# wdas03/lipreading-video-generation

Measured on AMD Instinct MI355X. Metric: train-step frames/sec + DDIM steps/sec, 128x128x16 UNet3D at 1/2/4/8 GPUs, higher is better.
Workload: dtype bf16

## Files before the change

### include/vdiff.h

```cpp
#ifndef VDIFF_H
#define VDIFF_H

#include <stdint.h>
#include <stddef.h>

#ifdef __cplusplus
extern "C" {
#endif

#define VDIFF_ABI_VERSION 1

enum vd_status { VD_OK = 0, VD_EINVAL = 1, VD_EUNSUPPORTED = 2, VD_ELAUNCH = 3 };
enum vd_dtype { VD_F32 = 0, VD_BF16 = 1 };

int vd_version(void);
const char* vd_last_error(void);
int vd_device_info(char* buf, int buflen);

int vd_timestep_embedding(const int64_t* t, int B, int dim, float max_period,
                          float* out, void* stream);
int vd_timestep_embedding_tab(const int64_t* t, int B, int dim, const float* freqs,
                              float* out, void* stream);

int vd_q_sample(const void* x0, const void* eps, void* xt, const int64_t* t,
                const float* sqrt_acp, const float* sqrt_1m_acp,
                int64_t B, int64_t per_sample, int dtype, void* stream);

// ... 16 lines not shown
                   int64_t B, int64_t per_sample, int dtype, void* stream);

int vd_p_sample_cosine(const void* xt, const void* eps, const void* z,
                       void* x_prev, void* mean_out, const int64_t* t,
                       const float* acp, const float* sqrt_acp,
                       const float* sqrt_1m_acp, int64_t B, int64_t per_sample,
                       int dtype, void* stream);

int vd_ddim_step(const void* xt, const void* eps, const void* z, void* x_prev,
                 void* x0, const int64_t* t, const int64_t* t_prev,
                 const float* acp, float eta, int clip, int64_t B,
                 int64_t per_sample, int dtype, void* stream);

void vd_set_dropout_counter(const uint64_t* counter);
int vd_groupnorm_set_unroll(int u);
size_t vd_groupnorm_workspace_size(int B, int64_t S, int C, int G);
int vd_groupnorm_silu_fwd(const void* x, const float* gamma, const float* beta,
                          void* y, float* mean, float* rstd, int B, int64_t S,
                          int C, int G, float eps, int silu, float drop_p,
                          uint64_t seed, int dtype, void* workspace,
                          void* stream);
int vd_groupnorm_silu_bwd(const void* x, const void* dy, const float* gamma,
                          const float* beta, const float* mean,
                          const float* rstd, void* dx, float* dgamma,
                          float* dbeta, int B, int64_t S, int C, int G,
                          int silu, float drop_p, uint64_t seed, int dtype,
                          void* workspace, void* stream);
int vd_groupnorm_silu_bwd_add(const void* x, const void* dy, const void* dadd,
                              const float* gamma, const float* beta, const float* mean,
                              const float* rstd, void* dx, float* dgamma, float* dbeta,
// ... 30 lines not shown
  int dtype;
} vd_conv_desc;

int vd_conv3d_fwd(const vd_conv_desc* d, const void* x, const void* w_fwd,
                  const float* bias, const float* chan_add,
                  const void* residual, void* y, void* stream);
int vd_conv3d_bwd_data(const vd_conv_desc* d, const void* dy,
                       const void* w_bwd, void* dx, void* stream);
int vd_conv3d_bwd_weight(const vd_conv_desc* d, const void* x, const void* dy,
                         float* dw, void* stream);
size_t vd_conv3d_bwd_weight_workspace_size(const vd_conv_desc* d);
int vd_conv3d_bwd_weight_det(const vd_conv_desc* d, const void* x, const void* dy, float* dw,
                             int Co_out, int Ci_out, void* workspace, size_t workspace_bytes,
                             void* stream);

int vd_conv_set_wgrad(int mode);
int vd_conv_set_halo(int mode);

size_t vd_channel_sums_workspace_size(int B, int C);
int vd_channel_sums(const void* x, int B, int64_t S, int C, int cstride, int dtype,
                    float* out, void* workspace, void* stream);
int vd_conv_pack_weight(const float* w, int Co, int Ci, int taps, int Cip, int Cop,
                        int transpose, int dtype, void* out, void* stream);
typedef struct {
  const float* w;
  void* out;
  int Co, Ci, taps, Cip, Cop, transpose;
  int64_t start;
} vd_pack_desc;
int vd_conv_pack_weights(const vd_pack_desc* descs, int n, int64_t total, int dtype,
                         void* stream);

// ... 76 lines not shown
```

### lipreading-video-generation_amd/csrc/conv.hip

```cpp
#include "vd_common.h"
#include <stdio.h>
#include <stdlib.h>

#include <atomic>

namespace {

constexpr int kThreads = 256;
constexpr int kBK = 32;

template <typename T> struct Cfg;
template <> struct Cfg<bf16_t> {
  static constexpr int EPC = 8;
  static constexpr int CPR = kBK / EPC;
  static constexpr int LDK = kBK;
};
template <> struct Cfg<float> {
  static constexpr int EPC = 4;
  static constexpr int CPR = kBK / EPC;
  static constexpr int LDK = kBK + 4;
};

__device__ __forceinline__ int swz(int r, int kc) {
  const int t = (r >> 2) & 3;
// ... 1700 lines not shown
int halo_ks(const GemmGeom& g, bool ) {
  if (conv_halo_mode() == 0 || !halo_ok(g)) return 0;
  static const int force = [] {
    const char* e = getenv("VDIFF_CONV_HALO_KS");
    return e ? atoi(e) : 0;
  }();
  if (force == 32 || force == 64) return force;
  return (g.dW <= 32 || g.sC >= 128) ? 64 : 32;
}
template <bool TR, int KS, int NW, bool EA = true, bool EH = false>
void launch_halo_tile(const GemmGeom& g, const void* src, const void* wt, void* dst,
                  const float* bias, const float* ca, const void* res, hipStream_t st) {
  const size_t lds_c = (size_t)kHoT * NW * kHoW * (64 + 4) * 4;
  const size_t lds = halo_lds<3, KS, NW>() > lds_c ? halo_lds<3, KS, NW>() : lds_c;
  auto kern = halo_conv_kernel<TR, KS, NW, EA, EH>;
  (void)hipFuncSetAttribute((const void*)kern, hipFuncAttributeMaxDynamicSharedMemorySize,
                            (int)lds);
  const int64_t tiles = (int64_t)g.B * vd_cdiv(g.dT, kHoT) * vd_cdiv(g.dH, NW) * (g.dW / kHoW);
  dim3 grid((unsigned)tiles, (unsigned)vd_cdiv(g.N, 64));
  kern<<<grid, 64 * NW, lds, st>>>(g, (const bf16_t*)src, (const bf16_t*)wt, (bf16_t*)dst, bias,
                                   ca, (const bf16_t*)res);
}
template <bool TR>
void launch_halo(const GemmGeom& g, int ks, const void* src, const void* wt, void* dst,
                 const float* bias, const float* ca, const void* res, hipStream_t st) {
  if (conv_halo_mode() == 3) {
    if (ks == 32) launch_halo_tile<TR, 32, 8>(g, src, wt, dst, bias, ca, res, st);
    else launch_halo_tile<TR, 64, 8>(g, src, wt, dst, bias, ca, res, st);
    return;
  }
  if (conv_halo_mode() == 4) {
    if (ks == 32) launch_halo_tile<TR, 32, 4, false>(g, src, wt, dst, bias, ca, res, st);
// ... 1 lines not shown
    return;
  }
  if constexpr (!TR) {
    if (conv_halo_mode() != 5) {
      if (ks == 32) launch_halo_tile<TR, 32, 4, true, true>(g, src, wt, dst, bias, ca, res, st);
      else launch_halo_tile<TR, 64, 4, true, true>(g, src, wt, dst, bias, ca, res, st);
      return;
    }
  }
  if (ks == 32) launch_halo_tile<TR, 32, 4>(g, src, wt, dst, bias, ca, res, st);
  else launch_halo_tile<TR, 64, 4>(g, src, wt, dst, bias, ca, res, st);
}

constexpr int kPwMaxLds = 40 * 1024;

template <int KS>
__global__ __launch_bounds__(256) void pw_gemm_kernel(
    const bf16_t* __restrict__ src, int sCs, const bf16_t* __restrict__ wt, int N, int NS,
    bf16_t* __restrict__ dst, int dNs, const float* __restrict__ bias,
    const float* __restrict__ chan_add, int64_t ppb, const bf16_t* __restrict__ residual,
    int64_t M) {
  constexpr int K = 32 * KS, RS = K + 8;
  extern __shared__ __attribute__((aligned(16))) char smem[];
  bf16_t* wl = reinterpret_cast<bf16_t*>(smem);
  const int tid = threadIdx.x, lane = tid & 63;
  const int wave = __builtin_amdgcn_readfirstlane(tid >> 6);
  const int nbase = blockIdx.y * NS;
  const int nsl = N - nbase < NS ? N - nbase : NS;
  const int nrow = (nsl + 63) / 64 * 64;
  for (int c = tid; c < nrow * (K / 8); c += 256) {
    const int r = c / (K / 8), k8 = c % (K / 8);
    *reinterpret_cast<uint4*>(wl + r * RS + k8 * 8) =
        r < nsl ? *reinterpret_cast<const uint4*>(wt + (int64_t)(nbase + r) * K + k8 * 8)
                : make_uint4(0, 0, 0, 0);
  }
  __syncthreads();

  const int fr = lane & 15, fq = lane >> 4;
  const int64_t ntiles = (M + 15) / 16;
  const int64_t stride = (int64_t)gridDim.x * 4;
  auto load = [&](bf16x8 (&x)[KS], int64_t tile) __attribute__((always_inline)) {
    const int64_t p = tile * 16 + fr;
    const bool ok = tile < ntiles && p < M;
    const bf16_t* row = src + (ok ? p : 0) * (int64_t)sCs + 8 * fq;
#pragma unroll
    for (int kk = 0; kk < KS; ++kk) {
      const uint4 v = ok ? *reinterpret_cast<const uint4*>(row + 32 * kk) : make_uint4(0, 0, 0, 0);
      x[kk] = __builtin_bit_cast(bf16x8, v);
    }
  };
  bf16x8 xc[KS], xn[KS];
  int64_t tile = (int64_t)blockIdx.x * 4 + wave;
  load(xc, tile);
  for (; tile < ntiles; tile += stride) {
    load(xn, tile + stride);
    const int64_t p = tile * 16 + fr;
    const bool pok = p < M;
    const int b = chan_add ? (int)((pok ? p : 0) / ppb) : 0;
    bf16_t* out = dst + (pok ? p : 0) * (int64_t)dNs + nbase;
    const bf16_t* res = residual ? residual + (pok ? p : 0) * (int64_t)dNs + nbase : nullptr;
    for (int n0 = 0; n0 < nsl; n0 += 64) {
      f32x4 acc[4];
#pragma unroll
      for (int j = 0; j < 4; ++j) acc[j] = f32x4{0.f, 0.f, 0.f, 0.f};
#pragma unroll
      for (int j = 0; j < 4; ++j) {
        const bf16_t* wr = wl + (n0 + 16 * (fr >> 2) + 4 * j + (fr & 3)) * RS + 8 * fq;
#pragma unroll
// ... 32 lines not shown
#pragma unroll
            for (int e = 0; e < 8; ++e) o[8 * h + e] += rv[e];
          }
        }
#pragma unroll
        for (int h = 0; h < 2; ++h) {
          float v8[8];
#pragma unroll
          for (int e = 0; e < 8; ++e) v8[e] = o[8 * h + e];
          store8(out + nl + 8 * h, v8);
        }
      }
    }
#pragma unroll
    for (int kk = 0; kk < KS; ++kk) xc[kk] = xn[kk];
  }
}

int pw_gemm_launch(const GemmGeom& g, const void* src, const void* wt, void* dst,
                   const float* bias, const float* ca, const void* res, hipStream_t st) {
  const int K = g.sC;
  if (g.kt * g.kh * g.kw != 1 || g.st != 1 || g.sh != 1 || g.sw != 1 || g.pt || g.ph || g.pw)
    return -1;
  if (K % 32 || K > 256 || g.N % 16 || g.sCs % 8 || g.dNs % 8 || g.K != K) return -1;
  if ((reinterpret_cast<uintptr_t>(src) & 15) || (reinterpret_cast<uintptr_t>(wt) & 15) ||
      (reinterpret_cast<uintptr_t>(dst) & 15) || (reinterpret_cast<uintptr_t>(res) & 15))
    return -1;
  if (bias && (reinterpret_cast<uintptr_t>(bias) & 15)) return -1;
  if (ca && ((reinterpret_cast<uintptr_t>(ca) & 15) || g.N % 4)) return -1;
  const int row_bytes = (K + 8) * 2;
  int NS = (kPwMaxLds / row_bytes) / 64 * 64;
  if (NS < 64) return -1;
  int slices = (int)vd_cdiv(g.N, NS);
  NS = (int)vd_cdiv(vd_cdiv(g.N, slices), 64) * 64;
  slices = (int)vd_cdiv(g.N, NS);
  const size_t lds = (size_t)NS * row_bytes;
  const int64_t tiles = vd_cdiv(g.M, 16);
  int64_t wgs = vd_cdiv(tiles, 4);
  const int64_t cap = (int64_t)256 * 4 / slices;
  if (wgs > cap) wgs = cap < 256 ? 256 : cap;
  const int64_t ppb = (int64_t)g.dT * g.dH * g.dW;
  dim3 grid((unsigned)wgs, (unsigned)slices);
#define VD_PW_CASE(KS_)                                                                          \
  case KS_: {                                                                                    \
    auto kern = pw_gemm_kernel<KS_>;                                                             \
    (void)hipFuncSetAttribute((const void*)kern, hipFuncAttributeMaxDynamicSharedMemorySize,     \
                              (int)lds);                                                         \
    kern<<<grid, 256, lds, st>>>((const bf16_t*)src, g.sCs, (const bf16_t*)wt, g.N, NS,          \
                                 (bf16_t*)dst, g.dNs, bias, ca, ppb, (const bf16_t*)res, g.M);   \
    return VD_OK;                                                                                \
  }
  switch (K / 32) {
    VD_PW_CASE(1) VD_PW_CASE(2) VD_PW_CASE(3) VD_PW_CASE(4)
    VD_PW_CASE(5) VD_PW_CASE(6) VD_PW_CASE(7) VD_PW_CASE(8)
  }
#undef VD_PW_CASE
  return -1;
}

#ifndef VD_PW_DEFAULT
#define VD_PW_DEFAULT 1
#endif
const bool g_conv_pw = [] {
  const char* e = getenv("VDIFF_CONV_PW");
  return e ? atoi(e) != 0 : VD_PW_DEFAULT != 0;
}();

int conv_1x1_variant() {
  static const int v = [] {
    const char* e = getenv("VDIFF_CONV_1X1");
    return e ? atoi(e) : 3;
// ... 103 lines not shown
  VD_REQUIRE(x && w_fwd && y, "null tensor");
  GemmGeom g;
  g.B = d->B;
  g.sT = d->Ti; g.sH = d->Hi; g.sW = d->Wi; g.sC = d->Ci;
  g.sCs = d->x_cstride ? d->x_cstride : d->Ci;
  g.dT = d->To; g.dH = d->Ho; g.dW = d->Wo; g.N = d->Co;
  g.dNs = d->y_cstride ? d->y_cstride : d->Co;
  g.kt = d->kt; g.kh = d->kh; g.kw = d->kw;
  g.st = d->st; g.sh = d->sh; g.sw = d->sw;
  g.pt = d->pt; g.ph = d->ph; g.pw = d->pw;
  g.M = (int64_t)d->B * d->To * d->Ho * d->Wo;
  g.K = d->kt * d->kh * d->kw * d->Ci;
  return VD_DISPATCH_DTYPE(d->dtype, T, {
    launch_gemm<T, false>(g, x, w_fwd, y, bias, chan_add, residual, VD_STREAM(stream));
  });
}

int vd_conv_set_wgrad(int mode) {
  if (mode < 0 || mode > 2) {
    (void)vd::fail(VD_EINVAL, "conv wgrad mode %d (0, 1, 2)", mode);
    return -2;
  }
  return g_wgrad_mode.exchange(mode);
}

int vd_conv_set_halo(int mode) {
  if (mode < 0 || mode > 5) {
    (void)vd::fail(VD_EINVAL, "conv halo mode %d (0 - 5)", mode);
    return -2;
  }
// ... 345 lines not shown
```

### lipreading-video-generation_amd/csrc/groupnorm.hip

```cpp
#include <atomic>

#include "vd_common.h"

namespace {

constexpr int kThreads = 256;
constexpr int kVec = 8;
static int env_int(const char* name, int dflt) {
  const char* e = getenv(name);
  const int v = e ? atoi(e) : 0;
  return v > 0 ? v : dflt;
}
const int kTargetChunks = env_int("VDIFF_GN_CHUNKS", 1024);
const int kSumPer = env_int("VDIFF_GN_SUMPER", 64);
std::atomic<int> g_gn_unroll{env_int("VDIFF_GN_UNROLL", 2)};

struct GNPlan {
  int rows_per_iter;
  int64_t chunk_px;
  int nchunk;
};

inline GNPlan gn_plan(int B, int64_t S, int C) {
  GNPlan p;
  const int nvec = C / kVec;
  p.rows_per_iter = kThreads / nvec;
  if (p.rows_per_iter < 1) p.rows_per_iter = 1;
  int64_t want = vd_cdiv(S * B, kTargetChunks);
  if (want < p.rows_per_iter) want = p.rows_per_iter;
  want = vd_cdiv(want, p.rows_per_iter) * p.rows_per_iter;
  p.chunk_px = want;
  p.nchunk = (int)vd_cdiv(S, want);
  return p;
}

struct Stat {
  float n, m, q;
};
__device__ __forceinline__ Stat chan(Stat a, Stat b) {
  const float n = a.n + b.n;
  if (n == 0.f) return a;
  const float d = b.m - a.m;
  const float fb = b.n / n;
  Stat r;
  r.n = n;
  r.m = a.m + d * fb;
  r.q = a.q + b.q + d * d * a.n * fb;
  return r;
}

struct Drop {
  float p, inv_keep;
  uint64_t seed;
  const uint64_t* ctr;
  __device__ __forceinline__ Drop resolved() const {
    Drop d = *this;
    if (p > 0.f && ctr) d.seed = seed ^ ((*ctr + 1) * 0x9E3779B97F4A7C15ull);
    d.ctr = nullptr;
    return d;
  }
  __device__ __forceinline__ float mul(int64_t idx) const {
    return p > 0.f ? dropout_mul(seed, idx, p, inv_keep) : 1.f;
  }
};
// ... 126 lines not shown
                                                            const float* __restrict__ beta,
                                                            const float* __restrict__ mean,
                                                            const float* __restrict__ rstd,
                                                            T* __restrict__ y, int64_t S, int C,
                                                            int G, int64_t chunk_px,
                                                            int rows_per_iter, Drop drop_in) {
  const Drop drop = drop_in.resolved();
  const int nvec = C / kVec, cpg = C / G;
  const int b = blockIdx.y, tid = threadIdx.x;
  const int r = tid / nvec, cv = tid % nvec;
  if (r >= rows_per_iter) return;
  float sc[kVec], sh[kVec];
#pragma unroll
  for (int j = 0; j < kVec; ++j) {
    const int c = cv * kVec + j, g = b * G + c / cpg;
    sc[j] = gamma[c] * rstd[g];
    sh[j] = beta[c] - mean[g] * sc[j];
  }
  const int64_t p0 = (int64_t)blockIdx.x * chunk_px;
  int64_t p1 = p0 + chunk_px;
  if (p1 > S) p1 = S;
  int64_t p = p0 + r;
  if constexpr (U > 1) {
    for (; p + (U - 1) * rows_per_iter < p1; p += U * rows_per_iter) {
      float v[U][kVec];
#pragma unroll
      for (int u = 0; u < U; ++u)
        load8(x + ((int64_t)b * S + p + u * rows_per_iter) * C + cv * kVec, v[u]);
#pragma unroll
      for (int u = 0; u < U; ++u) {
        const int64_t e0 = ((int64_t)b * S + p + u * rows_per_iter) * C + cv * kVec;
#pragma unroll
        for (int j = 0; j < kVec; ++j) {
          const float z = v[u][j] * sc[j] + sh[j];
          v[u][j] = (SILU ? silu_f(z) : z) * drop.mul(e0 + j);
        }
        store8(y + e0, v[u]);
      }
    }
  }
  for (; p < p1; p += rows_per_iter) {
    const int64_t e0 = ((int64_t)b * S + p) * C + cv * kVec;
    float v[kVec];
    load8(x + e0, v);
#pragma unroll
    for (int j = 0; j < kVec; ++j) {
      const float z = v[j] * sc[j] + sh[j];
      v[j] = (SILU ? silu_f(z) : z) * drop.mul(e0 + j);
    }
    store8(y + e0, v);
  }
}

template <typename T, bool SILU, int U>
__global__ __launch_bounds__(kThreads) void gn_bwd_reduce_kernel(
    const T* __restrict__ x, const T* __restrict__ dy, const float* __restrict__ gamma,
    const float* __restrict__ beta, const float* __restrict__ mean, const float* __restrict__ rstd,
    int64_t S, int C, int G, int64_t chunk_px, int rows_per_iter, float* __restrict__ part,
    Drop drop_in) {
  const Drop drop = drop_in.resolved();
  extern __shared__ __attribute__((aligned(16))) char smem[];
  float2* sh = reinterpret_cast<float2*>(smem);
// ... 220 lines not shown
}


int gn_check(const void* x, int B, int64_t S, int C, int G) {
  VD_REQUIRE(x, "null tensor");
  VD_REQUIRE(B > 0 && S > 0 && C > 0 && G > 0, "bad shape B=%d S=%lld C=%d G=%d", B,
             (long long)S, C, G);
  VD_REQUIRE(C % G == 0, "C=%d not divisible by groups=%d", C, G);
  VD_REQUIRE(C % kVec == 0, "C=%d must be a multiple of %d", C, kVec);
  VD_REQUIRE(C / kVec <= kThreads, "C=%d too large", C);
  VD_REQUIRE(G <= kThreads, "G=%d too large", G);
  VD_REQUIRE(C <= 4 * kThreads, "C=%d too large for bwd finalize", C);
  return VD_OK;
}

}

extern "C" {

size_t vd_groupnorm_workspace_size(int B, int64_t S, int C, int G) {
  if (B <= 0 || S <= 0 || C <= 0 || G <= 0 || C % kVec) return 0;
  GNPlan p = gn_plan(B, S, C);
  size_t fwd = (size_t)B * p.nchunk * G * 3 * sizeof(float);
  const size_t ksplit = vd_cdiv(p.nchunk, kSumPer);
  size_t bwd = ((size_t)B * p.nchunk * C * 2 + (size_t)B * G * 2 + ksplit * B * C * 2) *
               sizeof(float);
  return (fwd > bwd ? fwd : bwd) + 256;
}

void vd_set_dropout_counter(const uint64_t* counter) { g_drop_ctr = counter; }
// ... 32 lines not shown
  else                                                                                           \
    gn_apply_kernel<T, false, U><<<grid, kThreads, 0, st>>>((const T*)x, gamma, beta, mean,     \
                                                            rstd, (T*)y, S, C, G, p.chunk_px,   \
                                                            p.rows_per_iter, drop)
  const int u = g_gn_unroll.load(std::memory_order_relaxed);
  return VD_DISPATCH_DTYPE(dtype, T, {
    if (u == 4) {
      VD_GN_FWD(4);
    } else if (u == 2) {
      VD_GN_FWD(2);
    } else {
      VD_GN_FWD(1);
    }
  });
#undef VD_GN_FWD
}

int vd_groupnorm_silu_bwd(const void* x, const void* dy, const float* gamma, const float* beta,
                          const float* mean, const float* rstd, void* dx, float* dgamma,
                          float* dbeta, int B, int64_t S, int C, int G, int silu, float drop_p,
                          uint64_t seed, int dtype, void* workspace, void* stream) {
  return vd_groupnorm_silu_bwd_add(x, dy, nullptr, gamma, beta, mean, rstd, dx, dgamma, dbeta, B,
                                   S, C, G, silu, drop_p, seed, dtype, workspace, stream);
}

int vd_groupnorm_silu_bwd_add(const void* x, const void* dy, const void* dadd, const float* gamma,
                              const float* beta, const float* mean, const float* rstd, void* dx,
                              float* dgamma, float* dbeta, int B, int64_t S, int C, int G,
                              int silu, float drop_p, uint64_t seed, int dtype, void* workspace,
                              void* stream) {
// ... 50 lines not shown
```

### lipreading-video-generation_amd/csrc/vd_common.h

```cpp
#pragma once
#include <hip/hip_runtime.h>
#include <stdint.h>
#include <stddef.h>
#include "../../include/vdiff.h"

namespace vd {
void set_error(const char* fmt, ...);
int fail(int code, const char* fmt, ...);
int check_launch(const char* what);
}

#define VD_REQUIRE(cond, ...)                                   \
  do {                                                          \
    if (!(cond)) return vd::fail(VD_EINVAL, __VA_ARGS__);       \
  } while (0)

#define VD_STREAM(s) (reinterpret_cast<hipStream_t>(s))

typedef uint16_t bf16_t;
typedef short bf16x8 __attribute__((ext_vector_type(8)));
typedef short bf16x4 __attribute__((ext_vector_type(4)));
typedef float f32x4 __attribute__((ext_vector_type(4)));
typedef float f32x16 __attribute__((ext_vector_type(16)));
typedef __attribute__((address_space(3))) bf16x4 lds_bf16x4;
// ... 108 lines not shown
```

### lipreading-video-generation_amd/vdiff/_lib.py

```python
from __future__ import annotations

import ctypes as C
import os
import threading

_HERE = os.path.dirname(os.path.abspath(__file__))
LIB_PATH = os.environ.get("VDIFF_LIB") or os.path.join(_HERE, "libvdiff.so")

VD_F32 = 0
VD_BF16 = 1
ABI_VERSION = 1

_vp = C.c_void_p
_i = C.c_int
_i64 = C.c_int64
_u64 = C.c_uint64
_f = C.c_float
_sz = C.c_size_t


class ConvDesc(C.Structure):
    _fields_ = [(n, _i) for n in (
        "B", "Ti", "Hi", "Wi", "Ci", "To", "Ho", "Wo", "Co",
        "kt", "kh", "kw", "st", "sh", "sw", "pt", "ph", "pw",
        "x_cstride", "y_cstride", "dtype")]
# ... 13 lines not shown

_SIGS = {
    "vd_version": (_i, []),
    "vd_last_error": (C.c_char_p, []),
    "vd_device_info": (_i, [C.c_char_p, _i]),
    "vd_timestep_embedding": (_i, [_vp, _i, _i, _f, _vp, _vp]),
    "vd_timestep_embedding_tab": (_i, [_vp, _i, _i, _vp, _vp, _vp]),
    "vd_q_sample": (_i, [_vp, _vp, _vp, _vp, _vp, _vp, _i64, _i64, _i, _vp]),
    "vd_p_sample_v1": (_i, [_vp, _vp, _vp, _vp, _vp, _vp, _vp, _vp, _vp, _vp, _i64, _i64, _i, _vp]),
    "vd_p_sample_v2": (_i, [_vp, _vp, _vp, _vp, _vp, _vp, _vp, _vp, _vp, _vp, _vp, _i64, _i64, _i,
                            _vp]),
    "vd_p_sample_cosine": (_i, [_vp, _vp, _vp, _vp, _vp, _vp, _vp, _vp, _vp, _i64, _i64, _i, _vp]),
    "vd_ddim_step": (_i, [_vp, _vp, _vp, _vp, _vp, _vp, _vp, _vp, _f, _i, _i64, _i64, _i, _vp]),
    "vd_set_dropout_counter": (None, [_vp]),
    "vd_groupnorm_set_unroll": (_i, [_i]),
    "vd_groupnorm_workspace_size": (_sz, [_i, _i64, _i, _i]),
    "vd_groupnorm_silu_fwd": (_i, [_vp, _vp, _vp, _vp, _vp, _vp, _i, _i64, _i, _i, _f, _i, _f,
                                   _u64, _i, _vp, _vp]),
    "vd_groupnorm_silu_bwd": (_i, [_vp, _vp, _vp, _vp, _vp, _vp, _vp, _vp, _vp, _i, _i64, _i, _i,
                                   _i, _f, _u64, _i, _vp, _vp]),
    "vd_groupnorm_silu_bwd_add": (_i, [_vp, _vp, _vp, _vp, _vp, _vp, _vp, _vp, _vp, _vp, _i, _i64,
                                       _i, _i, _i, _f, _u64, _i, _vp, _vp]),
    "vd_silu": (_i, [_vp, _vp, _i64, _i, _vp]),
    "vd_silu_bwd": (_i, [_vp, _vp, _vp, _i64, _i, _vp]),
    "vd_cond_concat": (_i, [_vp, _vp, _vp, _vp, _i, _i, _i, _i, _i, _i, _i, _i, _i, _i, _i, _vp]),
    "vd_cond_concat_bwd_workspace_size": (_sz, [_i, _i, _i, _i, _i]),
    "vd_cond_concat_bwd": (_i, [_vp, _vp, _vp, _i, _i, _i, _i, _i, _i, _i, _i, _i, _i, _i, _vp,
                                _vp]),
    "vd_upsample_nearest_hw": (_i, [_vp, _vp, _i, _i, _i, _i, _i, _i, _vp]),
    "vd_upsample_nearest_hw_bwd": (_i, [_vp, _vp, _i, _i, _i, _i, _i, _i, _vp]),
    "vd_channel_sums_workspace_size": (_sz, [_i, _i]),
    "vd_channel_sums": (_i, [_vp, _i, _i64, _i, _i, _i, _vp, _vp, _vp]),
    "vd_conv_pack_weight": (_i, [_vp, _i, _i, _i, _i, _i, _i, _i, _vp, _vp]),
    "vd_conv_pack_weights": (_i, [_vp, _i, _i64, _i, _vp]),
    "vd_conv_set_wgrad": (_i, [C.c_int]),
    "vd_conv_set_halo": (_i, [_i]),
    "vd_conv3d_fwd": (_i, [C.POINTER(ConvDesc), _vp, _vp, _vp, _vp, _vp, _vp, _vp]),
    "vd_conv3d_bwd_data": (_i, [C.POINTER(ConvDesc), _vp, _vp, _vp, _vp]),
    "vd_conv3d_bwd_weight": (_i, [C.POINTER(ConvDesc), _vp, _vp, _vp, _vp]),
    "vd_conv3d_bwd_weight_workspace_size": (_sz, [C.POINTER(ConvDesc)]),
    "vd_conv3d_bwd_weight_det": (_i, [C.POINTER(ConvDesc), _vp, _vp, _vp, _i, _i, _vp, _sz, _vp]),
    "vd_attention_fwd": (_i, [C.POINTER(AttnDesc), _vp, _vp, _vp, _vp, _vp, _vp]),
    "vd_attention_fwd_workspace_size": (_sz, [C.POINTER(AttnDesc)]),
    "vd_attention_fwd_ws": (_i, [C.POINTER(AttnDesc), _vp, _vp, _vp, _vp, _vp, _vp, _sz, _vp]),
    "vd_attention_bwd_workspace_size": (_sz, [C.POINTER(AttnDesc)]),
    "vd_attention_set_config": (C.c_int, [C.c_int]),
    "vd_attention_bwd": (_i, [C.POINTER(AttnDesc), _vp, _vp, _vp, _vp, _vp, _vp, _vp, _vp, _vp,
                              _vp, _vp]),
    "vd_attention_bwd_dq": (_i, [C.POINTER(AttnDesc), _vp, _vp, _vp, _vp, _vp, _vp, _vp, _vp,
                                 _vp]),
    "vd_attention_bwd_dkdv": (_i, [C.POINTER(AttnDesc), _vp, _vp, _vp, _vp, _vp, _vp, _vp, _vp,
                                   _vp]),
# ... 65 lines not shown
```

### lipreading-video-generation_amd/vdiff/nn.py

```python
from __future__ import annotations

import math
from abc import abstractmethod

import torch as th
import torch.nn as nn
import torch.utils.checkpoint

from . import ops

ATTENTION_MODES = ("joint", "spatial", "temporal", "spatial_temporal")


class SiLU(nn.SiLU):

    def forward(self, x):
        return ops.silu(x)


class GroupNorm32(nn.GroupNorm):

    def forward(self, x):
        return ops.group_norm_silu(x, self.weight, self.bias, self.num_groups, self.eps,
                                   silu=False)
# ... 282 lines not shown
            self.temporal_proj_out = zero_module(conv_nd(1, channels, channels, 1))
        self.audio_attention = audio_attention
        self.audio_per_frame = audio_per_frame
        if audio_attention:
            self.audio_norm = normalization(channels)
            self.audio_q = conv_nd(1, channels, channels, 1)
            self.audio_kv = linear(audio_context_dim, 2 * channels)
            self.audio_proj_out = zero_module(conv_nd(1, channels, channels, 1))

    def forward(self, x, context=None):
        if context is None:
            return checkpoint(self._forward, (x,), self.parameters(), self.use_checkpoint)
        return checkpoint(self._forward, (x, context), self.parameters(), self.use_checkpoint)

    def _attend(self, xf, norm, qkv_conv, proj, mode, spatial):
        h, xs = ops.group_norm_silu_pass(xf, norm.weight, norm.bias, norm.num_groups, norm.eps,
                                         silu=False)
        qkv = ops.conv(h, qkv_conv.weight, qkv_conv.bias)
        a = ops.attention(qkv, self.num_heads, mode=mode, spatial=spatial, legacy=self.legacy)
        return ops.conv(a, proj.weight, proj.bias, residual=xs)

    def _cross(self, h, context, frames):
        a = ops.group_norm_silu(h, self.audio_norm.weight, self.audio_norm.bias,
                                self.audio_norm.num_groups, self.audio_norm.eps, silu=False)
        q = ops.conv(a, self.audio_q.weight, self.audio_q.bias)
        kv = ops.linear(context.to(h.dtype), self.audio_kv.weight, self.audio_kv.bias)
        o = ops.cross_attention(q, kv, self.num_heads, frames, self.audio_per_frame)
        return ops.conv(o, self.audio_proj_out.weight, self.audio_proj_out.bias, residual=h)

    def _forward(self, x, context=None):
        b, c, *spatial = x.shape
        x = ops.to_cl(x)
        xf = x.reshape(b, c, -1)
# ... 151 lines not shown
```

### lipreading-video-generation_amd/vdiff/ops.py

```python
from __future__ import annotations

import math
import os
from typing import Optional, Sequence, Tuple

import torch

from . import _lib
from ._lib import AttnDesc, ConvDesc, VD_BF16, VD_F32, XAttnDesc

_DT = {torch.float32: VD_F32, torch.bfloat16: VD_BF16}
_WGRAD_ATOMIC = os.environ.get("VDIFF_WGRAD_ATOMIC", "0") == "1"


def _p(t: Optional[torch.Tensor]):
    return None if t is None else t.data_ptr()


def _stream(t: torch.Tensor):
    return torch.cuda.current_stream(t.device).cuda_stream


def _dtype(t: torch.Tensor) -> int:
    try:
# ... 198 lines not shown

def group_norm_silu(x, weight, bias, groups=32, eps=1e-5, silu=True, dropout=0.0, seed=None):
    if dropout > 0.0 and seed is None:
        seed = new_seed()
    return GroupNormSiLUFn.apply(x, weight, bias, groups, eps, silu, float(dropout),
                                 int(seed or 0))


def group_norm_silu_pass(x, weight, bias, groups=32, eps=1e-5, silu=True):
    if not _GN_PASSTHROUGH:
        return group_norm_silu(x, weight, bias, groups, eps, silu), x
    return GroupNormSiLUFn.apply(x, weight, bias, groups, eps, silu, 0.0, 0, True)


_GN_PASSTHROUGH = os.environ.get("VDIFF_GN_PASSTHROUGH", "1") != "0"


class SiLUFn(torch.autograd.Function):
    @staticmethod
    def forward(ctx, x):
        _gpu(x)
        x = x.contiguous()
        y = torch.empty_like(x)
        _lib.call("vd_silu", _p(x), _p(y), x.numel(), _dtype(x), _stream(x))
        ctx.save_for_backward(x)
        return y

    @staticmethod
    def backward(ctx, dy):
        (x,) = ctx.saved_tensors
# ... 366 lines not shown
        parts.append(o)
    return torch.cat(parts, dim=1)[:, :Cc]


def _conv_key(Ci, Co, k, s, out):
    return f"{Ci}->{Co} k{'x'.join(map(str, k))} s{'x'.join(map(str, s))} out{'x'.join(map(str, out))}"


def _conv_flop(B, out, Co, k, Ci):
    return 2.0 * B * out[0] * out[1] * out[2] * Co * k[0] * k[1] * k[2] * Ci


class ConvFn(torch.autograd.Function):

    @staticmethod
    def forward(ctx, x, weight, bias, chan_add, residual, stride, padding):
        _gpu(x, weight)
        x = to_cl(x)
        dt = x.dtype
        Co, Ci = weight.shape[:2]
        if x.shape[1] != Ci:
            raise ValueError(f"conv expects {Ci} input channels, got {x.shape[1]}")
        nd, k, s, p, sp, out = _geom(x.shape, weight.shape, stride, padding)
        B = x.shape[0]
        taps = k[0] * k[1] * k[2]
        Cip = (Ci + 7) // 8 * 8
        xp = _pad_channels(x, Cip)
        w_fwd = _pack_weight(weight, Co, Ci, taps, Cip, Co, False, dt)
        ys = [B, Co] + out[3 - nd:] if nd > 0 else [B, Co]
        y = empty_cl(ys, dt, x.device)
        b32 = None if bias is None else bias.detach().float().contiguous()
        ca = None if chan_add is None else chan_add.detach().float().reshape(B, Co).contiguous()
        res = None
        if residual is not None:
            res = to_cl(residual).to(dt)
            if list(res.shape) != ys:
                raise ValueError(f"residual shape {list(res.shape)} != output {ys}")
        d = _desc(B, sp, Cip, out, Co, k, s, p, _DT[dt])
        ev = _timer.begin() if _timer is not None and _timer.convs else None
        _lib.call("vd_conv3d_fwd", d, _p(xp), _p(w_fwd), _p(b32), _p(ca), _p(res), _p(y),
                  _stream(x))
        if ev is not None:
            _timer.end_conv(ev, "conv_fwd", _conv_key(Cip, Co, k, s, out),
                            _conv_flop(B, out, Co, k, Ci))
        ctx.save_for_backward(xp, weight)
        ctx.cfg = (k, s, p, sp, out, B, Ci, Cip, Co, nd, list(x.shape), bias is not None,
                   chan_add is not None, residual is not None,
                   None if chan_add is None else chan_add.shape,
                   None if bias is None else bias.dtype)
        return y

    @staticmethod
    def backward(ctx, dy):
        xp, weight = ctx.saved_tensors
        (k, s, p, sp, out, B, Ci, Cip, Co, nd, xshape, has_b, has_ca, has_res, ca_shape,
         bdt) = ctx.cfg
# ... 37 lines not shown
                          _p(ws), ws.numel(), st)
            if ev is not None:
                _timer.end_conv(ev, "conv_bwd_weight", _conv_key(Cip, Co, k, s, out),
                                _conv_flop(B, out, Co, k, Ci))
            dw = dw.to(weight.dtype)
        want_b = has_b and ctx.needs_input_grad[2]
        want_ca = has_ca and ctx.needs_input_grad[3]
        if want_b or want_ca:
            sums = channel_sums(dyp)[:, :Co]
            if want_b:
                db = (sums[0] if B == 1 else sums.sum(0)).to(bdt)
            if want_ca:
                dca = sums.reshape(ca_shape)
        if has_res and ctx.needs_input_grad[4]:
            dres = dy
        return dx, dw, db, dca, dres, None, None


def conv(x, weight, bias=None, stride=1, padding=0, chan_add=None, residual=None):
    nd = weight.dim() - 2
    if isinstance(stride, int):
        stride = (stride,) * nd
    if isinstance(padding, int):
        padding = (padding,) * nd
    return ConvFn.apply(x, weight, bias, chan_add, residual, tuple(stride), tuple(padding))


class KernelTimer:

    def __init__(self, attention=True, convs=True):
        self.attention, self.convs = attention, convs
# ... 248 lines not shown
```

Before: 46.97.

## Fuse GroupNorm apply into pointwise QKV conv prologue for inference attention

Adds a GN-fused variant of the pointwise GEMM conv kernel. It builds per-channel scale/shift tables in LDS from precomputed group stats and normalizes input tiles on load, so the normalized tensor is never written out and read back. In no-grad attention blocks the QKV conv now uses a stats-only GroupNorm pass followed by this fused conv. The change also caches the hipFuncSetAttribute LDS-limit call per device instead of issuing it on every launch. The GN table consumes LDS, which may shrink the N slice per block.

New measurement: 46.84. Within noise of the previous version (-0.3%).

```diff
diff --git a/include/vdiff.h b/include/vdiff.h
--- a/include/vdiff.h
+++ b/include/vdiff.h
@@ -11,6 +11,7 @@
 #define VDIFF_ABI_VERSION 1
 
 enum vd_status { VD_OK = 0, VD_EINVAL = 1, VD_EUNSUPPORTED = 2, VD_ELAUNCH = 3 };
+#define VD_NOT_FUSED (-1)
 enum vd_dtype { VD_F32 = 0, VD_BF16 = 1 };
 
 int vd_version(void);
@@ -57,6 +58,9 @@
 
 void vd_set_dropout_counter(const uint64_t* counter);
 int vd_groupnorm_set_unroll(int u);
+int vd_groupnorm_set_fused(int on);
+int vd_groupnorm_stats(const void* x, float* mean, float* rstd, int B, int64_t S, int C, int G,
+                       float eps, int dtype, void* workspace, void* stream);
 size_t vd_groupnorm_workspace_size(int B, int64_t S, int C, int G);
 int vd_groupnorm_silu_fwd(const void* x, const float* gamma, const float* beta,
                           void* y, float* mean, float* rstd, int B, int64_t S,
@@ -117,8 +121,14 @@
                              int Co_out, int Ci_out, void* workspace, size_t workspace_bytes,
                              void* stream);
 
+int vd_conv_set_halo(int mode);
 int vd_conv_set_wgrad(int mode);
-int vd_conv_set_halo(int mode);
+
+int vd_conv3d_fwd_gn(const vd_conv_desc* d, const void* x, const float* gn_mean,
+                     const float* gn_rstd, const float* gn_gamma, const float* gn_beta, int G,
+                     const void* w_fwd, const float* bias, const float* chan_add,
+                     const void* residual, void* y, void* stream);
+int vd_conv3d_fwd_gn_fuses(const vd_conv_desc* d, int G);
 
 size_t vd_channel_sums_workspace_size(int B, int C);
 int vd_channel_sums(const void* x, int B, int64_t S, int C, int cstride, int dtype,
diff --git a/lipreading-video-generation_amd/csrc/conv.hip b/lipreading-video-generation_amd/csrc/conv.hip
--- a/lipreading-video-generation_amd/csrc/conv.hip
+++ b/lipreading-video-generation_amd/csrc/conv.hip
@@ -1,13 +1,27 @@
+#include "gn_common.h"
 #include "vd_common.h"
 #include <stdio.h>
 #include <stdlib.h>
 
 #include <atomic>
+#include <type_traits>
 
 namespace {
 
 constexpr int kThreads = 256;
 constexpr int kBK = 32;
+
+struct LdsLimitOnce {
+  std::atomic<uint64_t> done{0};
+  void raise(const void* kern, int bytes) {
+    int dev = 0;
+    (void)hipGetDevice(&dev);
+    const uint64_t bit = 1ull << (dev & 63);
+    if (done.load(std::memory_order_acquire) & bit) return;
+    (void)hipFuncSetAttribute(kern, hipFuncAttributeMaxDynamicSharedMemorySize, bytes);
+    done.fetch_or(bit, std::memory_order_release);
+  }
+};
 
 template <typename T> struct Cfg;
 template <> struct Cfg<bf16_t> {
@@ -1738,8 +1752,8 @@
   const size_t lds_c = (size_t)kHoT * NW * kHoW * (64 + 4) * 4;
   const size_t lds = halo_lds<3, KS, NW>() > lds_c ? halo_lds<3, KS, NW>() : lds_c;
   auto kern = halo_conv_kernel<TR, KS, NW, EA, EH>;
-  (void)hipFuncSetAttribute((const void*)kern, hipFuncAttributeMaxDynamicSharedMemorySize,
-                            (int)lds);
+  static LdsLimitOnce once;
+  once.raise((const void*)kern, (int)lds);
   const int64_t tiles = (int64_t)g.B * vd_cdiv(g.dT, kHoT) * vd_cdiv(g.dH, NW) * (g.dW / kHoW);
   dim3 grid((unsigned)tiles, (unsigned)vd_cdiv(g.N, 64));
   kern<<<grid, 64 * NW, lds, st>>>(g, (const bf16_t*)src, (const bf16_t*)wt, (bf16_t*)dst, bias,
@@ -1771,15 +1785,30 @@
 
 constexpr int kPwMaxLds = 40 * 1024;
 
-template <int KS>
+struct PwGn {
+  const float *mean, *rstd, *gamma, *beta;
+  int G, nb;
+};
+struct PwNoGn {};
+
+template <int KS, bool GN = false>
 __global__ __launch_bounds__(256) void pw_gemm_kernel(
     const bf16_t* __restrict__ src, int sCs, const bf16_t* __restrict__ wt, int N, int NS,
     bf16_t* __restrict__ dst, int dNs, const float* __restrict__ bias,
     const float* __restrict__ chan_add, int64_t ppb, const bf16_t* __restrict__ residual,
-    int64_t M) {
+    int64_t M, std::conditional_t<GN, PwGn, PwNoGn> gn) {
   constexpr int K = 32 * KS, RS = K + 8;
   extern __shared__ __attribute__((aligned(16))) char smem[];
   bf16_t* wl = reinterpret_cast<bf16_t*>(smem);
+  [[maybe_unused]] float* tab = reinterpret_cast<float*>(smem + (size_t)NS * RS * 2);
+  if constexpr (GN) {
+    const int cpg = K / gn.G;
+    for (int i = threadIdx.x; i < gn.nb * K; i += 256) {
+      const int c = i % K, g = (i / K) * gn.G + c / cpg;
+      vd_gn::scale_shift(gn.gamma[c], gn.beta[c], gn.mean[g], gn.rstd[g], tab[i],
+                         tab[gn.nb * K + i]);
+    }
+  }
   const int tid = threadIdx.x, lane = tid & 63;
   const int wave = __builtin_amdgcn_readfirstlane(tid >> 6);
   const int nbase = blockIdx.y * NS;
@@ -1806,9 +1835,35 @@
       x[kk] = __builtin_bit_cast(bf16x8, v);
     }
   };
+  [[maybe_unused]] auto norm = [&](bf16x8 (&x)[KS], int64_t t) __attribute__((always_inline)) {
+    if constexpr (GN) {
+      const int b = gn.nb > 1 && t < ntiles ? (int)(t * 16 / ppb) : 0;
+      const float* sc = tab + b * K + 8 * fq;
+      const float* sh = sc + gn.nb * K;
+#pragma unroll
+      for (int kk = 0; kk < KS; ++kk) {
+        const uint4 r = __builtin_bit_cast(uint4, x[kk]);
+        const uint32_t w[4] = {r.x, r.y, r.z, r.w};
+        float s[8], h[8], z[8];
+        *reinterpret_cast<float4*>(s) = *reinterpret_cast<const float4*>(sc + 32 * kk);
+        *reinterpret_cast<float4*>(s + 4) = *reinterpret_cast<const float4*>(sc + 32 * kk + 4);
+        *reinterpret_cast<float4*>(h) = *reinterpret_cast<const float4*>(sh + 32 * kk);
+        *reinterpret_cast<float4*>(h + 4) = *reinterpret_cast<const float4*>(sh + 32 * kk + 4);
+#pragma unroll
+        for (int i = 0; i < 4; ++i) {
+          z[2 * i] = vd_gn::apply(__uint_as_float(w[i] << 16), s[2 * i], h[2 * i]);
+          z[2 * i + 1] = vd_gn::apply(__uint_as_float(w[i] & 0xffff0000u), s[2 * i + 1],
+                                      h[2 * i + 1]);
+        }
+        x[kk] = __builtin_bit_cast(bf16x8, make_uint4(pack2bf(z[0], z[1]), pack2bf(z[2], z[3]),
+                                                      pack2bf(z[4], z[5]), pack2bf(z[6], z[7])));
+      }
+    }
+  };
   bf16x8 xc[KS], xn[KS];
   int64_t tile = (int64_t)blockIdx.x * 4 + wave;
   load(xc, tile);
+  norm(xc, tile);
   for (; tile < ntiles; tile += stride) {
     load(xn, tile + stride);
     const int64_t p = tile * 16 + fr;
@@ -1871,11 +1926,13 @@
     }
 #pragma unroll
     for (int kk = 0; kk < KS; ++kk) xc[kk] = xn[kk];
+    norm(xc, tile + stride);
   }
 }
 
 int pw_gemm_launch(const GemmGeom& g, const void* src, const void* wt, void* dst,
-                   const float* bias, const float* ca, const void* res, hipStream_t st) {
+                   const float* bias, const float* ca, const void* res, hipStream_t st,
+                   const PwGn* gn = nullptr, bool dry = false) {
   const int K = g.sC;
   if (g.kt * g.kh * g.kw != 1 || g.st != 1 || g.sh != 1 || g.sw != 1 || g.pt || g.ph || g.pw)
     return -1;
@@ -1885,26 +1942,38 @@
     return -1;
   if (bias && (reinterpret_cast<uintptr_t>(bias) & 15)) return -1;
   if (ca && ((reinterpret_cast<uintptr_t>(ca) & 15) || g.N % 4)) return -1;
+  const int64_t ppb = (int64_t)g.dT * g.dH * g.dW;
+  size_t tab = 0;
+  if (gn) {
+    if (gn->G <= 0 || K % gn->G || ppb % 16 || (int64_t)gn->nb * K > 1024) return -1;
+    tab = (size_t)2 * gn->nb * K * sizeof(float);
+  }
   const int row_bytes = (K + 8) * 2;
-  int NS = (kPwMaxLds / row_bytes) / 64 * 64;
+  int NS = (int)((kPwMaxLds - tab) / row_bytes) / 64 * 64;
   if (NS < 64) return -1;
   int slices = (int)vd_cdiv(g.N, NS);
   NS = (int)vd_cdiv(vd_cdiv(g.N, slices), 64) * 64;
   slices = (int)vd_cdiv(g.N, NS);
-  const size_t lds = (size_t)NS * row_bytes;
+  if (dry) return VD_OK;
+  const size_t lds = (size_t)NS * row_bytes + tab;
   const int64_t tiles = vd_cdiv(g.M, 16);
   int64_t wgs = vd_cdiv(tiles, 4);
   const int64_t cap = (int64_t)256 * 4 / slices;
   if (wgs > cap) wgs = cap < 256 ? 256 : cap;
-  const int64_t ppb = (int64_t)g.dT * g.dH * g.dW;
   dim3 grid((unsigned)wgs, (unsigned)slices);
+#define VD_PW_LAUNCH(KS_, GN_, ...)                                                              \
+  do {                                                                                           \
+    auto kern = pw_gemm_kernel<KS_, GN_>;                                                        \
+    static LdsLimitOnce once;                                                                    \
+    once.raise((const void*)kern, kPwMaxLds);                                                    \
+    kern<<<grid, 256, lds, st>>>((const bf16_t*)src, g.sCs, (const bf16_t*)wt, g.N, NS,          \
+                                 (bf16_t*)dst, g.dNs, bias, ca, ppb, (const bf16_t*)res, g.M,    \
+                                 __VA_ARGS__);                                                   \
+  } while (0)
 #define VD_PW_CASE(KS_)                                                                          \
   case KS_: {                                                                                    \
-    auto kern = pw_gemm_kernel<KS_>;                                                             \
-    (void)hipFuncSetAttribute((const void*)kern, hipFuncAttributeMaxDynamicSharedMemorySize,     \
-                              (int)lds);                                                         \
-    kern<<<grid, 256, lds, st>>>((const bf16_t*)src, g.sCs, (const bf16_t*)wt, g.N, NS,          \
-                                 (bf16_t*)dst, g.dNs, bias, ca, ppb, (const bf16_t*)res, g.M);   \
+    if (gn) VD_PW_LAUNCH(KS_, true, *gn);                                                        \
+    else VD_PW_LAUNCH(KS_, false, PwNoGn{});                                                     \
     return VD_OK;                                                                                \
   }
   switch (K / 32) {
@@ -1912,6 +1981,7 @@
     VD_PW_CASE(5) VD_PW_CASE(6) VD_PW_CASE(7) VD_PW_CASE(8)
   }
 #undef VD_PW_CASE
+#undef VD_PW_LAUNCH
   return -1;
 }
 
@@ -2045,6 +2115,47 @@
   return VD_DISPATCH_DTYPE(d->dtype, T, {
     launch_gemm<T, false>(g, x, w_fwd, y, bias, chan_add, residual, VD_STREAM(stream));
   });
+}
+
+static int conv_fwd_gn(const vd_conv_desc* d, const void* x, const float* gn_mean,
+                       const float* gn_rstd, const float* gn_gamma, const float* gn_beta, int G,
+                       const void* w_fwd, const float* bias, const float* chan_add,
+                       const void* residual, void* y, void* stream, bool dry) {
+  int rc = check_desc(d);
+  if (rc) return rc;
+  VD_REQUIRE(dry || (x && w_fwd && y && gn_mean && gn_rstd && gn_gamma && gn_beta),
+             "null tensor");
+  VD_REQUIRE(G > 0 && d->Ci % G == 0, "Ci=%d not divisible by groups=%d", d->Ci, G);
+  if (!vd::gn_fused() || d->dtype != VD_BF16 || g_legacy_conv || !g_conv_pw) return VD_NOT_FUSED;
+  GemmGeom g;
+  g.B = d->B;
+  g.sT = d->Ti; g.sH = d->Hi; g.sW = d->Wi; g.sC = d->Ci;
+  g.sCs = d->x_cstride ? d->x_cstride : d->Ci;
+  g.dT = d->To; g.dH = d->Ho; g.dW = d->Wo; g.N = d->Co;
+  g.dNs = d->y_cstride ? d->y_cstride : d->Co;
+  g.kt = d->kt; g.kh = d->kh; g.kw = d->kw;
+  g.st = d->st; g.sh = d->sh; g.sw = d->sw;
+  g.pt = d->pt; g.ph = d->ph; g.pw = d->pw;
+  g.M = (int64_t)d->B * d->To * d->Ho * d->Wo;
+  g.K = d->kt * d->kh * d->kw * d->Ci;
+  const PwGn gn{gn_mean, gn_rstd, gn_gamma, gn_beta, G, d->B};
+  if (pw_gemm_launch(g, x, w_fwd, y, bias, chan_add, residual, VD_STREAM(stream), &gn, dry) !=
+      VD_OK)
+    return VD_NOT_FUSED;
+  return dry ? VD_OK : vd::check_launch("vd_conv3d_fwd_gn");
+}
+
+int vd_conv3d_fwd_gn(const vd_conv_desc* d, const void* x, const float* gn_mean,
+                     const float* gn_rstd, const float* gn_gamma, const float* gn_beta, int G,
+                     const void* w_fwd, const float* bias, const float* chan_add,
+                     const void* residual, void* y, void* stream) {
+  return conv_fwd_gn(d, x, gn_mean, gn_rstd, gn_gamma, gn_beta, G, w_fwd, bias, chan_add, residual,
+                     y, stream, false);
+}
+
+int vd_conv3d_fwd_gn_fuses(const vd_conv_desc* d, int G) {
+  return conv_fwd_gn(d, nullptr, nullptr, nullptr, nullptr, nullptr, G, nullptr, nullptr, nullptr,
+                     nullptr, nullptr, nullptr, true);
 }
 
 int vd_conv_set_wgrad(int mode) {
diff --git a/lipreading-video-generation_amd/csrc/gn_common.h b/lipreading-video-generation_amd/csrc/gn_common.h
--- /dev/null
+++ b/lipreading-video-generation_amd/csrc/gn_common.h
@@ -0,0 +1,28 @@
+#pragma once
+#include "vd_common.h"
+
+namespace vd_gn {
+
+struct Stat {
+  float n, m, q;
+};
+__device__ __forceinline__ Stat chan(Stat a, Stat b) {
+  const float n = a.n + b.n;
+  if (n == 0.f) return a;
+  const float d = b.m - a.m;
+  const float fb = b.n / n;
+  Stat r;
+  r.n = n;
+  r.m = a.m + d * fb;
+  r.q = a.q + b.q + d * d * a.n * fb;
+  return r;
+}
+
+__device__ __forceinline__ void scale_shift(float gamma, float beta, float mean, float rstd,
+                                            float& sc, float& sh) {
+  sc = gamma * rstd;
+  sh = fmaf(-mean, sc, beta);
+}
+__device__ __forceinline__ float apply(float x, float sc, float sh) { return fmaf(x, sc, sh); }
+
+}
diff --git a/lipreading-video-generation_amd/csrc/groupnorm.hip b/lipreading-video-generation_amd/csrc/groupnorm.hip
--- a/lipreading-video-generation_amd/csrc/groupnorm.hip
+++ b/lipreading-video-generation_amd/csrc/groupnorm.hip
@@ -1,5 +1,6 @@
 #include <atomic>
 
+#include "gn_common.h"
 #include "vd_common.h"
 
 namespace {
@@ -14,6 +15,10 @@
 const int kTargetChunks = env_int("VDIFF_GN_CHUNKS", 1024);
 const int kSumPer = env_int("VDIFF_GN_SUMPER", 64);
 std::atomic<int> g_gn_unroll{env_int("VDIFF_GN_UNROLL", 2)};
+std::atomic<int> g_gn_fused{[] {
+  const char* e = getenv("VDIFF_GN_FUSED");
+  return e && atoi(e) == 0 && e[0] == '0' ? 0 : 1;
+}()};
 
 struct GNPlan {
   int rows_per_iter;
@@ -34,20 +39,8 @@
   return p;
 }
 
-struct Stat {
-  float n, m, q;
-};
-__device__ __forceinline__ Stat chan(Stat a, Stat b) {
-  const float n = a.n + b.n;
-  if (n == 0.f) return a;
-  const float d = b.m - a.m;
-  const float fb = b.n / n;
-  Stat r;
-  r.n = n;
-  r.m = a.m + d * fb;
-  r.q = a.q + b.q + d * d * a.n * fb;
-  return r;
-}
+using vd_gn::Stat;
+using vd_gn::chan;
 
 struct Drop {
   float p, inv_keep;
@@ -204,8 +197,7 @@
 #pragma unroll
   for (int j = 0; j < kVec; ++j) {
     const int c = cv * kVec + j, g = b * G + c / cpg;
-    sc[j] = gamma[c] * rstd[g];
-    sh[j] = beta[c] - mean[g] * sc[j];
+    vd_gn::scale_shift(gamma[c], beta[c], mean[g], rstd[g], sc[j], sh[j]);
   }
   const int64_t p0 = (int64_t)blockIdx.x * chunk_px;
   int64_t p1 = p0 + chunk_px;
@@ -222,7 +214,7 @@
         const int64_t e0 = ((int64_t)b * S + p + u * rows_per_iter) * C + cv * kVec;
 #pragma unroll
         for (int j = 0; j < kVec; ++j) {
-          const float z = v[u][j] * sc[j] + sh[j];
+          const float z = vd_gn::apply(v[u][j], sc[j], sh[j]);
           v[u][j] = (SILU ? silu_f(z) : z) * drop.mul(e0 + j);
         }
         store8(y + e0, v[u]);
@@ -235,7 +227,7 @@
     load8(x + e0, v);
 #pragma unroll
     for (int j = 0; j < kVec; ++j) {
-      const float z = v[j] * sc[j] + sh[j];
+      const float z = vd_gn::apply(v[j], sc[j], sh[j]);
       v[j] = (SILU ? silu_f(z) : z) * drop.mul(e0 + j);
     }
     store8(y + e0, v);
@@ -486,6 +478,10 @@
   return VD_OK;
 }
 
+}
+
+namespace vd {
+bool gn_fused() { return g_gn_fused.load(std::memory_order_relaxed) != 0; }
 }
 
 extern "C" {
@@ -548,6 +544,41 @@
     }
   });
 #undef VD_GN_FWD
+}
+
+int vd_groupnorm_set_fused(int on) {
+  if (on != 0 && on != 1) {
+    (void)vd::fail(VD_EINVAL, "groupnorm fused %d (0, 1)", on);
+    return -2;
+  }
+  return g_gn_fused.exchange(on);
+}
+
+int vd_groupnorm_stats(const void* x, float* mean, float* rstd, int B, int64_t S, int C, int G,
+                       float eps, int dtype, void* workspace, void* stream) {
+  int rc = gn_check(x, B, S, C, G);
+  if (rc) return rc;
+  VD_REQUIRE(mean && rstd && workspace, "null argument");
+  GNPlan p = gn_plan(B, S, C);
+  float* part = reinterpret_cast<float*>(workspace);
+  hipStream_t st = VD_STREAM(stream);
+  const size_t lds = (size_t)p.rows_per_iter * C * sizeof(Stat);
+  const dim3 grid(p.nchunk, B);
+#define VD_GN_STATS(U)                                                                          \
+  gn_stats_kernel<T, U><<<grid, kThreads, lds, st>>>((const T*)x, S, C, G, p.chunk_px,         \
+                                                     p.rows_per_iter, part);                   \
+  gn_finalize_kernel<<<dim3(G, B), kThreads, 0, st>>>(part, p.nchunk, G, eps, mean, rstd)
+  const int u = g_gn_unroll.load(std::memory_order_relaxed);
+  return VD_DISPATCH_DTYPE(dtype, T, {
+    if (u == 4) {
+      VD_GN_STATS(4);
+    } else if (u == 2) {
+      VD_GN_STATS(2);
+    } else {
+      VD_GN_STATS(1);
+    }
+  });
+#undef VD_GN_STATS
 }
 
 int vd_groupnorm_silu_bwd(const void* x, const void* dy, const float* gamma, const float* beta,
diff --git a/lipreading-video-generation_amd/csrc/vd_common.h b/lipreading-video-generation_amd/csrc/vd_common.h
--- a/lipreading-video-generation_amd/csrc/vd_common.h
+++ b/lipreading-video-generation_amd/csrc/vd_common.h
@@ -8,6 +8,7 @@
 void set_error(const char* fmt, ...);
 int fail(int code, const char* fmt, ...);
 int check_launch(const char* what);
+bool gn_fused();
 }
 
 #define VD_REQUIRE(cond, ...)                                   \
diff --git a/lipreading-video-generation_amd/vdiff/_lib.py b/lipreading-video-generation_amd/vdiff/_lib.py
--- a/lipreading-video-generation_amd/vdiff/_lib.py
+++ b/lipreading-video-generation_amd/vdiff/_lib.py
@@ -9,6 +9,7 @@
 
 VD_F32 = 0
 VD_BF16 = 1
+VD_NOT_FUSED = -1
 ABI_VERSION = 1
 
 _vp = C.c_void_p
@@ -52,6 +53,8 @@
     "vd_ddim_step": (_i, [_vp, _vp, _vp, _vp, _vp, _vp, _vp, _vp, _f, _i, _i64, _i64, _i, _vp]),
     "vd_set_dropout_counter": (None, [_vp]),
     "vd_groupnorm_set_unroll": (_i, [_i]),
+    "vd_groupnorm_set_fused": (_i, [_i]),
+    "vd_groupnorm_stats": (_i, [_vp, _vp, _vp, _i, _i64, _i, _i, _f, _i, _vp, _vp]),
     "vd_groupnorm_workspace_size": (_sz, [_i, _i64, _i, _i]),
     "vd_groupnorm_silu_fwd": (_i, [_vp, _vp, _vp, _vp, _vp, _vp, _i, _i64, _i, _i, _f, _i, _f,
                                    _u64, _i, _vp, _vp]),
@@ -74,6 +77,9 @@
     "vd_conv_set_wgrad": (_i, [C.c_int]),
     "vd_conv_set_halo": (_i, [_i]),
     "vd_conv3d_fwd": (_i, [C.POINTER(ConvDesc), _vp, _vp, _vp, _vp, _vp, _vp, _vp]),
+    "vd_conv3d_fwd_gn": (_i, [C.POINTER(ConvDesc), _vp, _vp, _vp, _vp, _vp, _i, _vp, _vp, _vp,
+                              _vp, _vp, _vp]),
+    "vd_conv3d_fwd_gn_fuses": (_i, [C.POINTER(ConvDesc), _i]),
     "vd_conv3d_bwd_data": (_i, [C.POINTER(ConvDesc), _vp, _vp, _vp, _vp]),
     "vd_conv3d_bwd_weight": (_i, [C.POINTER(ConvDesc), _vp, _vp, _vp, _vp]),
     "vd_conv3d_bwd_weight_workspace_size": (_sz, [C.POINTER(ConvDesc)]),
diff --git a/lipreading-video-generation_amd/vdiff/nn.py b/lipreading-video-generation_amd/vdiff/nn.py
--- a/lipreading-video-generation_amd/vdiff/nn.py
+++ b/lipreading-video-generation_amd/vdiff/nn.py
@@ -320,9 +320,14 @@
         return checkpoint(self._forward, (x, context), self.parameters(), self.use_checkpoint)
 
     def _attend(self, xf, norm, qkv_conv, proj, mode, spatial):
-        h, xs = ops.group_norm_silu_pass(xf, norm.weight, norm.bias, norm.num_groups, norm.eps,
-                                         silu=False)
-        qkv = ops.conv(h, qkv_conv.weight, qkv_conv.bias)
+        if ops.gn_fused() and not th.is_grad_enabled():
+            xs = xf
+            qkv = ops.conv_gn(xf, norm.weight, norm.bias, norm.num_groups, norm.eps,
+                              qkv_conv.weight, qkv_conv.bias)
+        else:
+            h, xs = ops.group_norm_silu_pass(xf, norm.weight, norm.bias, norm.num_groups,
+                                             norm.eps, silu=False)
+            qkv = ops.conv(h, qkv_conv.weight, qkv_conv.bias)
         a = ops.attention(qkv, self.num_heads, mode=mode, spatial=spatial, legacy=self.legacy)
         return ops.conv(a, proj.weight, proj.bias, residual=xs)
 
diff --git a/lipreading-video-generation_amd/vdiff/ops.py b/lipreading-video-generation_amd/vdiff/ops.py
--- a/lipreading-video-generation_amd/vdiff/ops.py
+++ b/lipreading-video-generation_amd/vdiff/ops.py
@@ -236,6 +236,33 @@
 
 
 _GN_PASSTHROUGH = os.environ.get("VDIFF_GN_PASSTHROUGH", "1") != "0"
+_GN_FUSED = os.environ.get("VDIFF_GN_FUSED", "1") != "0"
+
+
+def gn_fused() -> bool:
+    return _GN_FUSED
+
+
+def set_gn_fused(on: bool) -> bool:
+    global _GN_FUSED
+    prev = _GN_FUSED
+    _GN_FUSED = bool(on)
+    if _lib.lib().vd_groupnorm_set_fused(int(_GN_FUSED)) < 0:
+        raise RuntimeError("vd_groupnorm_set_fused failed")
+    return prev
+
+
+def group_norm_stats(x, groups=32, eps=1e-5):
+    _gpu(x)
+    x = to_cl(x)
+    B, Cc, S = x.shape[0], x.shape[1], _spatial(x)
+    mean = torch.empty(B * groups, dtype=torch.float32, device=x.device)
+    rstd = torch.empty_like(mean)
+    ws = torch.empty(_lib.lib().vd_groupnorm_workspace_size(B, S, Cc, groups),
+                     dtype=torch.uint8, device=x.device)
+    _lib.call("vd_groupnorm_stats", _p(x), _p(mean), _p(rstd), B, S, Cc, groups, float(eps),
+              _dtype(x), _p(ws), _stream(x))
+    return mean, rstd
 
 
 class SiLUFn(torch.autograd.Function):
@@ -632,7 +659,7 @@
 class ConvFn(torch.autograd.Function):
 
     @staticmethod
-    def forward(ctx, x, weight, bias, chan_add, residual, stride, padding):
+    def forward(ctx, x, weight, bias, chan_add, residual, stride, padding, gn=None):
         _gpu(x, weight)
         x = to_cl(x)
         dt = x.dtype
@@ -656,8 +683,11 @@
                 raise ValueError(f"residual shape {list(res.shape)} != output {ys}")
         d = _desc(B, sp, Cip, out, Co, k, s, p, _DT[dt])
         ev = _timer.begin() if _timer is not None and _timer.convs else None
-        _lib.call("vd_conv3d_fwd", d, _p(xp), _p(w_fwd), _p(b32), _p(ca), _p(res), _p(y),
-                  _stream(x))
+        if gn is not None:
+            xp = _conv_gn_input(d, xp, gn, w_fwd, b32, ca, res, y)
+        if xp is not None:
+            _lib.call("vd_conv3d_fwd", d, _p(xp), _p(w_fwd), _p(b32), _p(ca), _p(res), _p(y),
+                      _stream(x))
         if ev is not None:
             _timer.end_conv(ev, "conv_fwd", _conv_key(Cip, Co, k, s, out),
                             _conv_flop(B, out, Co, k, Ci))
@@ -725,7 +755,34 @@
                 dca = sums.reshape(ca_shape)
         if has_res and ctx.needs_input_grad[4]:
             dres = dy
-        return dx, dw, db, dca, dres, None, None
+        return dx, dw, db, dca, dres, None, None, None
+
+
+def _conv_gn_input(d, x, gn, w_fwd, b32, ca, res, y):
+    gw, gb, groups, eps = gn
+    g32 = gw.detach().float().contiguous()
+    be32 = gb.detach().float().contiguous()
+    if (_GN_FUSED and x.dtype == torch.bfloat16
+            and _lib.lib().vd_conv3d_fwd_gn_fuses(d, groups) == 0):
+        mean, rstd = group_norm_stats(x, groups, eps)
+        rc = _lib.lib().vd_conv3d_fwd_gn(d, _p(x), _p(mean), _p(rstd), _p(g32), _p(be32), groups,
+                                         _p(w_fwd), _p(b32), _p(ca), _p(res), _p(y), _stream(x))
+        if rc == 0:
+            return None
+        if rc != _lib.VD_NOT_FUSED:
+            _lib.check(rc, "vd_conv3d_fwd_gn")
+    return GroupNormSiLUFn.apply(x, g32, be32, groups, eps, False, 0.0, 0)
+
+
+def conv_gn(x, norm_weight, norm_bias, groups, eps, weight, bias=None):
+    if torch.is_grad_enabled():
+        raise RuntimeError("conv_gn keeps nothing for a backward: call it under torch.no_grad()")
+    nd = weight.dim() - 2
+    if weight.shape[1] % 8:
+        return conv(group_norm_silu(x, norm_weight, norm_bias, groups, eps, silu=False), weight,
+                    bias)
+    return ConvFn.apply(x, weight, bias, None, None, (1,) * nd, (0,) * nd,
+                        (norm_weight, norm_bias, int(groups), float(eps)))
 
 
 def conv(x, weight, bias=None, stride=1, padding=0, chan_add=None, residual=None):
```
